# barry-mir/mixing-style-transfer

Hardware: AMD Instinct MI355X
Metric: triplets/sec (10 s @ 44.1 kHz, 4-stem, bs=24) (higher is better)
Workload: dtype f32

## Files before the change

### mixing-style-transfer_amd/csrc/encoder.hip

```cpp
#include "common.h"

#include <cmath>
#include <type_traits>
#include <vector>

namespace {

typedef float f32x4 __attribute__((ext_vector_type(4)));
constexpr int kConvThreads = 512;
constexpr int kConvWaves = 8;

struct FilmParams {
  const float* feats;
  const float *w0t, *b0, *w3t, *b3, *hwt, *hb;
  const float *s1, *t1, *s2, *t2;
  float* film;
  float2* aff1;
  float2* aff2;
  int Fd, H, nsub;
  float* h2;
  int B;
};

constexpr int kFilmCT = 8;
// ... 689 lines not shown
  int nsaddr[4] = {-1, -1, -1, -1};

  auto prefetch_setup = [&](int q, const RTile& t) __attribute__((always_inline)) {
    const int chunk = q % NCH;
    const float* src = p.in + (size_t)t.clip * p.in_clipstride + (size_t)t.band * p.in_bandoff + (size_t)(4 * chunk) * p.in_cstride;
    const float* wsrc = p.wfrag + ((size_t)t.band * NCH + chunk) * WBP;
    nrsrc = __builtin_amdgcn_make_buffer_rsrc(const_cast<float*>(src), 0, (unsigned)(4 * p.in_cstride) * 4u, 0x00020000);
    nwrsrc = __builtin_amdgcn_make_buffer_rsrc(const_cast<float*>(wsrc), 0, (unsigned)WBP * 4u, 0x00020000);
    if (chunk == 0) {
      const bool fold = t.kind == 2;
      const int row0 = (t.kind == 1 ? 4 : 0) - 3, col0 = 16 * t.blk - 3;
      const int rbase = max(row0, 0), cbase = max(col0, 0);
      nsoff = (unsigned)(rbase * p.in_cols + cbase) * 4u;
      int ln = lane;
      asm volatile("" : "+v"(ln));
#pragma unroll
      for (int j = 0; j < 4; ++j) {
        const int e = ln + 64 * j;
        const int r = fold ? e >> 4 : e / PC, c = fold ? e & 15 : e % PC;
        const bool in_patch = fold ? (r < R::FR && c < R::FC) : r < R::PR;
        const int rin = row0 + r, cin = col0 + c;
        const bool ok = t.valid && in_patch && rin >= 0 && rin < p.in_rows && cin >= 0 && cin < p.in_cols;
        nvoff[j] = ok ? (unsigned)((rin - rbase) * p.in_cols + (cin - cbase)) * 4u : 0x80000000u;
        nsaddr[j] = in_patch ? r * PC + c : -1;
      }
    }
  };
  auto prefetch_piece = [&](int i) __attribute__((always_inline)) {
    if (i < NPFK) {
      pf[i] = __builtin_bit_cast(float, __builtin_amdgcn_raw_buffer_load_b32(nrsrc, nvoff[i & 3], nsoff + (unsigned)((i >> 2) * p.in_cstride) * 4u, 0));
    } else if (i < NPIECE) {
      wreg[i - NPFK] = __builtin_bit_cast(f32x4, __builtin_amdgcn_raw_buffer_load_b128(nwrsrc, (unsigned)tid * 16u, (unsigned)(kConvThreads * (i - NPFK)) * 16u, 0));
    }
  };

  f32x4 acc[MT][NT];
  RTile cur{}, nxt{};
  nxt = decode(0);
  if (nq > 0) {
    prefetch_setup(0, nxt);
#pragma unroll
    for (int i = 0; i < NPIECE; ++i) prefetch_piece(i);
  }
#ifdef MST_TRACE
  long long trc[5] = {0, 0, 0, 0, 0};
  const long long trc_start = clock64();
#endif
  for (int q = 0; q < nq; ++q) {
    float* wb = wbuf + (q & 1) * WBP;
#ifdef MST_TRACE
    const long long tq0 = clock64();
#endif
#pragma unroll
    for (int i = 0; i < NWF; ++i) reinterpret_cast<f32x4*>(wb)[tid + kConvThreads * i] = wreg[i];
#pragma unroll
    for (int i = 0; i < NPFK; ++i)
      if (nsaddr[i & 3] >= 0) pbuf[(i >> 2) * CP + nsaddr[i & 3]] = pf[i];
#ifdef MST_TRACE
    asm volatile("s_waitcnt lgkmcnt(0)" ::: "memory");
    const long long tq1 = clock64();
#endif
    __syncthreads();
#ifdef MST_TRACE
    const long long tq2 = clock64();
    trc[0] += tq1 - tq0, trc[1] += tq2 - tq1, trc[4] += 1;
#endif
    cur = nxt;
    if ((q + 1) % NCH == 0) nxt = decode(q + 1);
    prefetch_setup(q + 1, nxt);
    const int chunk = q % NCH;
    if (chunk == 0) {
      ap = cur.kind == 2 ? ap_fold : ap_pair;
#pragma unroll
      for (int t = 0; t < MT; ++t)
#pragma unroll
        for (int n = 0; n < NT; ++n) acc[t][n] = f32x4{0.f, 0.f, 0.f, 0.f};
    }
    {
      float a[2][MT], b[2][NT];
#pragma unroll
      for (int t = 0; t < MT; ++t) a[0][t] = ap[t * PC];
#pragma unroll
      for (int n = 0; n < NT; ++n) b[0][n] = wb[n * 64 + lane];
      auto taps = [&](auto LO_, auto HI_, auto MASK_) __attribute__((always_inline)) {
        constexpr int LO = decltype(LO_)::value, HI = decltype(HI_)::value, MASK = decltype(MASK_)::value;
#pragma unroll
        for (int tap = LO; tap < HI; ++tap) {
          const int cu = tap & 1, nx = cu ^ 1;
          const int off = ((tap + 1) / 7) * PC + ((tap + 1) % 7);
#pragma unroll
          for (int i = 0; i < MT * NT; ++i) {
            const int t = i / NT, n = i % NT;
            if (!((MASK >> t) & 1)) acc[t][n] = __builtin_amdgcn_mfma_f32_16x16x4f32(a[cu][t], b[cu][n], acc[t][n], 0, 0, 0);
            if (tap + 1 < 49) {
              if (i < NT) b[nx][i] = wb[((tap + 1) * NT + i) * 64 + lane];
              else if (i < MT + NT) a[nx][i - NT] = ap[(i - NT) * PC + off];
            }
            if (i >= MT + NT && i - (MT + NT) < PPT) prefetch_piece(tap * PPT + (i - (MT + NT)));
            __builtin_amdgcn_sched_barrier(0);
          }
        }
      };
      using std::integral_constant;
      using I0 = integral_constant<int, 0>;
      using I7 = integral_constant<int, 7>;
      using I14 = integral_constant<int, 14>;
      using I21 = integral_constant<int, 21>;
      using I42 = integral_constant<int, 42>;
      using I49 = integral_constant<int, 49>;
      if (cur.kind == 0) {
        taps(I0{}, I7{}, integral_constant<int, 0b0111>{});
        taps(I7{}, I14{}, integral_constant<int, 0b0011>{});
        taps(I14{}, I21{}, integral_constant<int, 0b0001>{});
      } else {
        taps(I0{}, I21{}, I0{});
      }
      taps(I21{}, I42{}, I0{});
      if (cur.kind == 1) taps(I42{}, I49{}, integral_constant<int, 0b1000>{});
      else taps(I42{}, I49{}, I0{});
    }
#ifdef MST_TRACE
    trc[2] += clock64() - tq2;
#endif
    if (chunk == NCH - 1 && cur.valid) {
      const int j = lane & 15, g = lane >> 4;
      const float2* aff = p.aff + ((size_t)cur.clip * p.nsub + cur.band) * C::COUT;
      const int pr = cur.kind == 2 ? g >> 1 : cur.kind;
      const int pc = 4 * cur.blk + (cur.kind == 2 ? g & 1 : g);
#pragma unroll
      for (int n = 0; n < NT; ++n) {
        const int ch = n * 16 + j;
        const float2 ac = aff[ch];
        float m = 0.f;
#pragma unroll
        for (int t = 0; t < MT; ++t)
#pragma unroll
          for (int r = 0; r < 4; ++r) m = fmaxf(m, fmaf(acc[t][n][r], ac.x, ac.y));
        if (pc < p.out_cols)
          p.out[(((size_t)cur.clip * p.nsub + cur.band) * C::COUT + ch) * p.out_rows * p.out_cols + (size_t)pr * p.out_cols + pc] = m;
      }
    }
  }
#ifdef MST_TRACE
  if (lane == 0 && p.yraw) {
    float* o = p.yraw + (blockIdx.x * kConvWaves + wave) * 8;
    for (int i = 0; i < 5; ++i) o[i] = (float)trc[i];
    o[5] = (float)(clock64() - trc_start);
  }
#endif
}

template <int SUB>
constexpr size_t kConv1ResidentLds = (size_t)(2 * 49 * CC<1, SUB>::NT * 64 + kConvWaves * 8 * CC<1, SUB>::PR * CC<1, SUB>::PC) * sizeof(float);
template <int SUB, int MODE = 0, int LAY = 0>
__global__ __launch_bounds__(kConvThreads) void conv1_resident_kernel(const ConvParams p) {
  using C = CC<1, SUB>;
  constexpr int MT = C::MT, NT = C::NT, PR = C::PR, PC = C::PC;
  static_assert(C::RL == 64, "resident conv1 expects one loader row per instruction");
  static_assert(LAY == 0 || PR == 8, "the channel-minor loader maps lane bits 1..3 to the 8 patch rows");
  constexpr int WCH = 49 * NT * 64;
  constexpr int WBP = ConvGeom<1, SUB>::WBP;
  constexpr int CHS = PR * PC;
  constexpr int PATCH = 8 * CHS;
  constexpr int NPF = LAY == 0 ? 8 * PR : (PC + 3) / 4;
  extern __shared__ __attribute__((aligned(16))) float smem[];
  const int tid = threadIdx.x, lane = tid & 63;
  const int wave = __builtin_amdgcn_readfirstlane(tid >> 6);
  float* wres = smem;
  float* pbuf = smem + 2 * WCH + wave * PATCH;
  constexpr bool DYN = MODE == 0;
  constexpr int kTickets = 16;
  __shared__ unsigned tickets[kTickets];
#ifdef MST_TRACE
  long long trc[5] = {0, 0, 0, 0, 0};
  const long long trc_start = clock64();
#endif

  const int G = gridDim.x;
  const int wg = mst::xcd_remap(blockIdx.x, G);
  const int total_sets = (p.clip_major ? (p.B + p.clip_major - 1) / p.clip_major : 1) * p.nsub * p.sets_per_band;
  const int s_begin = (int)((long long)wg * total_sets / G), s_end = (int)((long long)(wg + 1) * total_sets / G);
  const int tpb = p.tiles_r * p.tiles_c;

  auto decode = [&](int s) __attribute__((always_inline)) {
    Tile t;
    int ti;
    if (p.clip_major) {
      const int ngrp = (p.B + p.clip_major - 1) / p.clip_major;
      const int gb = min(s / p.sets_per_band, ngrp * p.nsub - 1);
      const int idx = (s - gb * p.sets_per_band) * kConvWaves + wave;
      const int grp = gb / p.nsub, c0 = grp * p.clip_major;
      t.band = gb - grp * p.nsub;
      t.valid = (s < s_end) && idx < min(p.clip_major, p.B - c0) * tpb;
      const int cl = t.valid ? idx / tpb : 0;
      t.clip = c0 + cl;
      ti = t.valid ? idx - cl * tpb : 0;
    } else {
      t.band = min(s / p.sets_per_band, p.nsub - 1);
      const int idx = (s - t.band * p.sets_per_band) * kConvWaves + wave;
      t.valid = (s < s_end) && idx < p.B * tpb;
      t.clip = t.valid ? idx / tpb : 0;
      ti = t.valid ? idx - t.clip * tpb : 0;
    }
    t.tc = ti / p.tiles_r;
    t.tr = ti - t.tc * p.tiles_r;
    return t;
  };

  const int kq = lane >> 4, ai = lane & 15, ag = ai >> 2, areg = ai & 3;
  int abase[MT];
#pragma unroll
  for (int t = 0; t < MT; ++t) {
    const int e = 4 * t + areg, wv = e / C::WIN, pos = e % C::WIN;
    abase[t] = kq * CHS + (pos / 5) * PC + 5 * (C::WPG * ag + wv) + pos % 5;
  }

  typename std::conditional<LAY == 0, float, f32x4>::type pf[NPF];
  unsigned long long rowmask = 0;
  bool col_ok = false;
  int coff = 0, nrow0 = 0, nvalid = 0;
  const float* nsrc = p.in;
  bool nfast = false;
  __amdgpu_buffer_rsrc_t nrsrc = __builtin_amdgcn_make_buffer_rsrc(const_cast<float*>(p.in), 0, 0, 0x00020000);
  unsigned nsoff = 0, nvoff = 0;
  static_assert(WBP - WCH >= 4, "the chunk pitch leaves at least 16 zero bytes behind the weights");
  const float* const zero16 = p.wfrag + WCH;
  const int lr = (lane >> 1) & 7, lhalf = lane & 1, lfq = lane >> 4;
  const unsigned frame_bytes = (unsigned)p.cm_mels * 32u;
  auto prefetch_setup = [&](const Tile& t) __attribute__((always_inline)) {
    nrow0 = C::TROWS * t.tr - 3;
    nvalid = t.valid;
    rowmask = 0;
    if constexpr (LAY == 0) {
      const int col0 = C::TCOLS * t.tc - 3, cin = col0 + lane;
      nsrc = p.in + (size_t)t.clip * p.in_clipstride + (size_t)t.band * p.in_bandoff;
      col_ok = lane < PC && cin >= 0 && cin < p.in_cols;
      coff = min(max(cin, 0), p.in_cols - 1);
    } else {
      const int rin = nrow0 + lr, rc = min(max(rin, 0), p.in_rows - 1);
      nsrc = p.in + (size_t)t.clip * p.in_clipstride;
      col_ok = nvalid && rin == rc;
      coff = ((t.band * p.cm_overlap + rc) * 8 + 4 * lhalf) * 4;
      nrow0 = C::TCOLS * t.tc - 3 + lfq;
      if constexpr (DYN) {
        const int f0 = C::TCOLS * t.tc - 3;
        nfast = nvalid && f0 >= 0 && f0 + 4 * NPF + 3 < p.in_cols;
        nrsrc = __builtin_amdgcn_make_buffer_rsrc(const_cast<float*>(nsrc), 0, (unsigned)p.in_cols * frame_bytes, 0x00020000);
        nsoff = (unsigned)max(f0, 0) * frame_bytes;
        nvoff = col_ok ? (unsigned)coff + (unsigned)lfq * frame_bytes : 0x80000000u;
      }
    }
  };
  auto prefetch_piece = [&](int i) __attribute__((always_inline)) {
    if (i < NPF) {
      if constexpr (LAY == 0) {
        const int cc = i / PR, r = i % PR;
        const int rin = nrow0 + r;
        const int rc = min(max(rin, 0), p.in_rows - 1);
        if (nvalid && rin == rc) rowmask |= 1ull << i;
        const float* rowp = nsrc + (size_t)cc * p.in_cstride + (size_t)rc * p.in_cols;
        if constexpr (DYN) pf[i] = (nvalid && rin == rc && col_ok) ? rowp[coff] : *zero16;
        else pf[i] = rowp[coff];
      } else {
        const int fin = nrow0 + 4 * i, fc = min(max(fin, 0), p.in_cols - 1);
        if (col_ok && fin == fc) rowmask |= 1ull << i;
        if (DYN && nfast) {
          pf[i] = __builtin_bit_cast(f32x4, __builtin_amdgcn_raw_buffer_load_b128(nrsrc, nvoff, nsoff + (unsigned)(4 * i) * frame_bytes, 0));
        } else {
          const unsigned boff = (unsigned)fc * frame_bytes + (unsigned)coff;
          const char* src = reinterpret_cast<const char*>(nsrc) + boff;
          if constexpr (DYN) src = (col_ok && fin == fc) ? src : reinterpret_cast<const char*>(zero16);
          pf[i] = *reinterpret_cast<const f32x4*>(src);
        }
      }
    }
  };
  auto prefetch_step = [&](int ks) __attribute__((always_inline)) {
    if constexpr (LAY == 0) prefetch_piece(ks);
    else if (ks % 8 == 0) prefetch_piece(ks / 8);
  };

  f32x4 acc[MT][NT];
  double st[NT][2];
#pragma unroll
  for (int n = 0; n < NT; ++n) st[n][0] = st[n][1] = 0.0;
  int cur_band = -1;
  const int spb = p.sets_per_band;
  const int gb0 = s_begin / spb, nseg = s_end > s_begin ? (s_end - 1) / spb - gb0 + 1 : 0;
  int dseg = 0, dlo = 0, dhi = 0, dgb = 0, nxt_seg = 0;
  auto seg_range = [&](int k) __attribute__((always_inline)) {
    dgb = gb0 + k;
    const int cm = p.clip_major ? p.clip_major : p.B, grp = p.clip_major ? dgb / p.nsub : 0;
    dlo = max(s_begin - dgb * spb, 0) * kConvWaves;
    dhi = min((min(s_end, (dgb + 1) * spb) - dgb * spb) * kConvWaves, min(cm, p.B - grp * cm) * tpb);
  };
  unsigned tkv = 0;
  auto ticket_issue = [&]() __attribute__((always_inline)) {
    tkv = 0;
    if (dseg < nseg && lane == 0)
      tkv = __hip_atomic_fetch_add(&tickets[dseg % kTickets], 1u, __ATOMIC_RELAXED, __HIP_MEMORY_SCOPE_WORKGROUP);
  };
  auto ticket_take = [&]() __attribute__((always_inline)) {
    Tile t{};
    while (dseg < nseg) {
      const int idx = dlo + (int)__builtin_amdgcn_readfirstlane(tkv);
      if (idx < dhi) {
        const int grp = p.clip_major ? dgb / p.nsub : 0;
        const int cl = idx / tpb, ti = idx - cl * tpb;
        t.valid = 1;
        t.band = dgb - grp * p.nsub;
        t.clip = grp * p.clip_major + cl;
        t.tc = ti / p.tiles_r;
        t.tr = ti - t.tc * p.tiles_r;
        return t;
      }
      if (++dseg < nseg) seg_range(dseg);
      ticket_issue();
    }
    return t;
  };
  Tile cur{}, nxt{};
  if constexpr (DYN) {
    if (tid < kTickets) tickets[tid] = 0;
    __syncthreads();
    if (nseg > 0) seg_range(0);
    ticket_issue();
    nxt = ticket_take();
    nxt_seg = dseg;
  } else {
    nxt = decode(s_begin);
  }
  prefetch_setup(nxt);
#pragma unroll
  for (int i = 0; i < NPF; ++i) prefetch_piece(i);

  auto mask_piece = [&](int i) __attribute__((always_inline)) {
    if constexpr (LAY == 0) {
      pf[i] = (((rowmask >> i) & 1ull) && col_ok) ? pf[i] : 0.f;
    } else {
      const bool ok = (rowmask >> i) & 1ull;
#pragma unroll
      for (int k = 0; k < 4; ++k) pf[i][k] = ok ? pf[i][k] : 0.f;
    }
  };
  auto stage_ = [&](auto MASKED_) __attribute__((always_inline)) {
    constexpr bool MASKED = decltype(MASKED_)::value;
    if constexpr (LAY == 0) {
#pragma unroll
      for (int i = 0; i < NPF; ++i) {
        if (!MASKED) mask_piece(i);
        if (lane < PC) pbuf[i * PC + lane] = pf[i];
      }
    } else {
      float* pl = pbuf + (4 * lhalf) * CHS + lr * PC + lfq;
#pragma unroll
      for (int i = 0; i < NPF; ++i) {
        if (4 * i + 3 < PC || 4 * i + lfq < PC) {
          if (!MASKED) mask_piece(i);
#pragma unroll
          for (int k = 0; k < 4; ++k) pl[k * CHS + 4 * i] = pf[i][k];
        }
      }
    }
  };
  auto stage = [&]() __attribute__((always_inline)) { stage_(std::false_type{}); };
  auto tile_body = [&]() __attribute__((always_inline)) {
#ifdef MST_TRACE
    const long long tr0 = clock64();
#endif
#pragma unroll
    for (int t = 0; t < MT; ++t)
#pragma unroll
      for (int n = 0; n < NT; ++n) acc[t][n] = f32x4{0.f, 0.f, 0.f, 0.f};
    {
      float a[2][MT], b[2][NT];
#pragma unroll
      for (int t = 0; t < MT; ++t) a[0][t] = pbuf[abase[t]];
#pragma unroll
      for (int n = 0; n < NT; ++n) b[0][n] = wres[n * 64 + lane];
#pragma unroll
      for (int ks = 0; ks < 98; ++ks) {
        const int cu = ks & 1, nx = cu ^ 1;
        const int tap = (ks + 1) >> 1, ch = (ks + 1) & 1;
        const int off = ch * 4 * CHS + (tap / 7) * PC + (tap % 7);
#pragma unroll
        for (int i = 0; i < MT * NT; ++i) {
          const int t = i / NT, n = i % NT;
          acc[t][n] = __builtin_amdgcn_mfma_f32_16x16x4f32(a[cu][t], b[cu][n], acc[t][n], 0, 0, 0);
          if (ks + 1 < 98) {
            if (i < NT) b[nx][i] = wres[ch * WCH + (tap * NT + i) * 64 + lane];
            else if (i < MT + NT) a[nx][i - NT] = pbuf[abase[i - NT] + off];
          }
          if (i == MT + NT) prefetch_step(ks);
          __builtin_amdgcn_sched_barrier(0);
        }
      }
    }
#ifdef MST_TRACE
    const long long tr1 = clock64();
    trc[0] += tr1 - tr0, trc[4] += 1;
#endif
    if constexpr (MODE == 1) {
      const int j = lane & 15, g = lane >> 4;
      float* yb = p.yraw + ((((size_t)cur.clip * p.nsub + cur.band) * p.acc_tr + cur.tr) * p.acc_tc + cur.tc) *
                               (size_t)(NT * 64 * 4 * MT);
#pragma unroll
      for (int n = 0; n < NT; ++n) {
        const float b = p.bias[cur.band * C::COUT + n * 16 + j];
        f32x4* dst = reinterpret_cast<f32x4*>(yb) + (size_t)n * (64 * MT) + lane;
#pragma unroll
        for (int t = 0; t < MT; ++t) {
          f32x4 v = acc[t][n];
#pragma unroll
          for (int r = 0; r < 4; ++r) {
            v[r] += b;
            const int e = 4 * t + r, wv = e / C::WIN, pos = e % C::WIN;
            const int col = C::TCOLS * cur.tc + 5 * (C::WPG * g + wv) + pos % 5;
            if (col < p.raw_cols) st[n][0] += (double)v[r], st[n][1] += (double)v[r] * (double)v[r];
          }
          dst[64 * t] = v;
        }
      }
    } else
    {
      const int j = lane & 15, g = lane >> 4;
      const float2* aff = p.aff + ((size_t)cur.clip * p.nsub + cur.band) * C::COUT;
      float* orow = p.out + ((size_t)cur.clip * p.nsub + cur.band) * C::COUT * p.out_rows * p.out_cols +
                    (size_t)cur.tr * p.out_cols;
#pragma unroll
      for (int n = 0; n < NT; ++n) {
        const int ch = n * 16 + j;
        const float2 ac = aff[ch];
#pragma unroll
        for (int wv = 0; wv < C::WPG; ++wv) {
          const int pc = 4 * C::WPG * cur.tc + C::WPG * g + wv;
          if (SUB == 2 && p.pool_h == 1) {
#pragma unroll
            for (int hr = 0; hr < 2; ++hr) {
              float m = 0.f;
#pragma unroll
              for (int pos = 0; pos < 5; ++pos) {
                const int e = wv * C::WIN + 5 * hr + pos;
                m = fmaxf(m, fmaf(acc[e >> 2][n][e & 3], ac.x, ac.y));
              }
              if (pc < p.out_cols && 2 * cur.tr + hr < p.out_rows)
                orow[(size_t)ch * p.out_rows * p.out_cols + (size_t)(cur.tr + hr) * p.out_cols + pc] = m;
            }
          } else {
            float m = 0.f;
#pragma unroll
            for (int pos = 0; pos < C::WIN; ++pos) {
              const int e = wv * C::WIN + pos;
              m = fmaxf(m, fmaf(acc[e >> 2][n][e & 3], ac.x, ac.y));
            }
            if (pc < p.out_cols) orow[(size_t)ch * p.out_rows * p.out_cols + pc] = m;
          }
        }
      }
    }
#ifdef MST_TRACE
    trc[1] += clock64() - tr1;
#endif
  };
  f32x4 sav[MT][NT];
  float2 sav_ac[NT];
  Tile prev{};
#pragma unroll
  for (int t = 0; t < MT; ++t)
#pragma unroll
    for (int n = 0; n < NT; ++n) sav[t][n] = f32x4{0.f, 0.f, 0.f, 0.f};
#pragma unroll
  for (int n = 0; n < NT; ++n) sav_ac[n] = float2{0.f, 0.f};
  auto epi_part = [&](auto N_, auto WV_) __attribute__((always_inline)) {
    constexpr int n = decltype(N_)::value, wv = decltype(WV_)::value;
    const int j = lane & 15, g = lane >> 4;
    const int ch = n * 16 + j;
    float* orow = p.out + ((size_t)prev.clip * p.nsub + prev.band) * C::COUT * p.out_rows * p.out_cols + (size_t)prev.tr * p.out_cols;
    const float2 ac = sav_ac[n];
    const int pc = 4 * C::WPG * prev.tc + C::WPG * g + wv;
    if (SUB == 2 && p.pool_h == 1) {
#pragma unroll
      for (int hr = 0; hr < 2; ++hr) {
        float m = 0.f;
#pragma unroll
        for (int pos = 0; pos < 5; ++pos) {
          const int e = wv * C::WIN + 5 * hr + pos;
          m = fmaxf(m, fmaf(sav[e >> 2][n][e & 3], ac.x, ac.y));
        }
        if (prev.valid && pc < p.out_cols && 2 * prev.tr + hr < p.out_rows)
          orow[(size_t)ch * p.out_rows * p.out_cols + (size_t)(prev.tr + hr) * p.out_cols + pc] = m;
      }
    } else {
      float m = 0.f;
#pragma unroll
      for (int pos = 0; pos < C::WIN; ++pos) {
        const int e = wv * C::WIN + pos;
        m = fmaxf(m, fmaf(sav[e >> 2][n][e & 3], ac.x, ac.y));
      }
      if (prev.valid && pc < p.out_cols) orow[(size_t)ch * p.out_rows * p.out_cols + pc] = m;
    }
  };
  auto tile_dyn = [&]() __attribute__((always_inline)) {
#ifdef MST_TRACE
    const long long tr0 = clock64();
#endif
    float2 e_ac[NT];
    {
      const float2* aff = p.aff + ((size_t)cur.clip * p.nsub + cur.band) * C::COUT;
#pragma unroll
      for (int n = 0; n < NT; ++n) e_ac[n] = aff[n * 16 + (lane & 15)];
    }
    {
      constexpr int kEpi0 = 12;
      const bool skip_c = cur.tr == 0, skip_b = 2 * cur.tr + 2 >= p.in_rows;
      const int next_off = skip_b ? 0 : 5 * PC, next_w = skip_b ? 0 : 35 * NT * 64;
      float a[2][MT], b[2][NT];
#pragma unroll
      for (int t = 0; t < MT; ++t) a[0][t] = pbuf[abase[t] + 2 * PC];
#pragma unroll
      for (int n = 0; n < NT; ++n) b[0][n] = wres[(14 * NT + n) * 64 + lane];
      auto kstep = [&](auto S_) __attribute__((always_inline)) {
        constexpr int ks = decltype(S_)::value;
        constexpr int cu = ks & 1, nx = cu ^ 1;
        constexpr bool last = ks == 41 || ks == 69 || ks == 97;
        constexpr int s1 = ks + 1, l1 = s1 < 42 ? s1 : s1 < 70 ? s1 - 42 : s1 - 70;
        constexpr int row1 = (s1 < 42 ? 2 : s1 < 70 ? 5 : 0) + l1 / 14, tap1 = 7 * row1 + (l1 % 14) / 2, ch1 = l1 & 1;
        constexpr int off1 = ch1 * 4 * CHS + row1 * PC + (l1 % 14) / 2;
#pragma unroll
        for (int i = 0; i < MT * NT; ++i) {
          const int t = i / NT, n = i % NT;
          acc[t][n] = __builtin_amdgcn_mfma_f32_16x16x4f32(a[cu][t], b[cu][n], ks == 0 ? f32x4{0.f, 0.f, 0.f, 0.f} : acc[t][n], 0, 0, 0);
          if constexpr (!last) {
            if (i < NT) b[nx][i] = wres[ch1 * WCH + (tap1 * NT + i) * 64 + lane];
            else if (i < MT + NT) a[nx][i - NT] = pbuf[abase[i - NT] + off1];
          } else if constexpr (ks == 41) {
            if (i < NT) b[nx][i] = wres[next_w + i * 64 + lane];
            else if (i < MT + NT) a[nx][i - NT] = pbuf[abase[i - NT] + next_off];
          } else if constexpr (ks == 69) {
            if (i < NT) b[nx][i] = wres[i * 64 + lane];
            else if (i < MT + NT) a[nx][i - NT] = pbuf[abase[i - NT]];
          }
          if (i == MT + NT) {
            if constexpr (LAY == 0) {
              if constexpr (ks >= 8 && ks < 8 + NPF / 2) prefetch_piece(2 * (ks - 8)), prefetch_piece(2 * (ks - 8) + 1);
            } else {
              if constexpr (ks >= 8 && ks % 2 == 0 && ks / 2 - 4 < NPF) prefetch_piece(ks / 2 - 4);
            }
          }
          if (i == MT + NT + 1) {
            if constexpr (ks == 0) ticket_issue();
            if constexpr (ks == 6) {
              nxt = ticket_take();
              nxt_seg = dseg;
              prefetch_setup(nxt);
            }
            if constexpr (ks >= kEpi0 && ks < kEpi0 + 2 * NT * C::WPG && (ks - kEpi0) % 2 == 0)
              epi_part(std::integral_constant<int, (ks - kEpi0) / 2 / C::WPG>{}, std::integral_constant<int, (ks - kEpi0) / 2 % C::WPG>{});
          }
          __builtin_amdgcn_sched_barrier(0);
        }
      };
      static_assert(LAY == 0 ? 8 + NPF / 2 <= 42 : 2 * (NPF + 3) < 42, "the patch fetch must fit block A");
      static_for<42>([&](auto I) __attribute__((always_inline)) { kstep(std::integral_constant<int, decltype(I)::value>{}); });
      if (!skip_b) static_for<28>([&](auto I) __attribute__((always_inline)) { kstep(std::integral_constant<int, 42 + decltype(I)::value>{}); });
      if (!skip_c) static_for<28>([&](auto I) __attribute__((always_inline)) { kstep(std::integral_constant<int, 70 + decltype(I)::value>{}); });
    }
    {
      const float bz = wres[lane];
#pragma unroll
      for (int t = 0; t < MT; ++t)
#pragma unroll
        for (int n = 0; n < NT; ++n) sav[t][n] = __builtin_amdgcn_mfma_f32_16x16x4f32(0.f, bz, acc[t][n], 0, 0, 0);
    }
#pragma unroll
    for (int n = 0; n < NT; ++n) sav_ac[n] = e_ac[n];
    prev = cur;
#ifdef MST_TRACE
    trc[0] += clock64() - tr0, trc[4] += 1;
#endif
  };
  auto load_band = [&](int band) __attribute__((always_inline)) {
    for (int c = 0; c < 2; ++c) {
      const f32x4* src = reinterpret_cast<const f32x4*>(p.wfrag + ((size_t)band * 2 + c) * WBP);
      for (int k = tid; k < WCH / 4; k += kConvThreads) reinterpret_cast<f32x4*>(wres + c * WCH)[k] = src[k];
    }
  };
  if constexpr (DYN) {
    for (int k = 0; k < nseg; ++k) {
#ifdef MST_TRACE
      const long long tb0 = clock64();
#endif
      __syncthreads();
      load_band((gb0 + k) % p.nsub);
      if (tid == 0) tickets[(k + kTickets - 1) % kTickets] = 0;
      __syncthreads();
#ifdef MST_TRACE
      trc[3] += clock64() - tb0;
#endif
      while (nxt.valid && nxt_seg == k) {
#ifdef MST_TRACE
        const long long ts0 = clock64();
#endif
        cur = nxt;
#ifdef MST_TRACE
        asm volatile("s_waitcnt vmcnt(0)" ::: "memory");
        const long long ts1 = clock64();
        trc[1] += ts1 - ts0;
#endif
        stage_(std::true_type{});
#ifdef MST_TRACE
        asm volatile("s_waitcnt lgkmcnt(0)" ::: "memory");
        trc[2] += clock64() - ts1;
#endif
        tile_dyn();
      }
    }
    {
      static_for<NT * C::WPG>([&](auto I) __attribute__((always_inline)) {
        constexpr int q = decltype(I)::value;
        epi_part(std::integral_constant<int, q / C::WPG>{}, std::integral_constant<int, q % C::WPG>{});
      });
    }
#ifdef MST_TRACE
    if (lane == 0 && p.yraw) {
      float* o = p.yraw + (blockIdx.x * kConvWaves + wave) * 8;
      for (int i = 0; i < 5; ++i) o[i] = (float)trc[i];
      o[5] = (float)(clock64() - trc_start);
    }
#endif
  } else {
  for (int s = s_begin; s < s_end; ++s) {
    cur = nxt;
    if (cur.band != cur_band) {
      if (MODE == 1 && cur_band >= 0) flush_stats<NT, C::COUT>(st, p.stats, cur_band, lane);
      __syncthreads();
      load_band(cur.band);
      __syncthreads();
      cur_band = cur.band;
    }
    stage();
    nxt = decode(s + 1);
    prefetch_setup(nxt);
    if (!cur.valid) {
#pragma unroll
      for (int i = 0; i < NPF; ++i) prefetch_piece(i);
      continue;
    }
    tile_body();
  }
  }
  if (MODE == 1 && cur_band >= 0) flush_stats<NT, C::COUT>(st, p.stats, cur_band, lane);
}

__global__ __launch_bounds__(256) void absmax_kernel(const float* __restrict__ x, long long n_per_clip, unsigned* out) {
  const float* base = x + (size_t)blockIdx.y * n_per_clip;
  float m = 0.f;
  const long long n4 = n_per_clip >> 2;
  const float4* b4 = reinterpret_cast<const float4*>(base);
  const bool al = (reinterpret_cast<uintptr_t>(base) & 15) == 0;
  if (al) {
    for (long long i = (long long)blockIdx.x * 256 + threadIdx.x; i < n4; i += (long long)gridDim.x * 256) {
      const float4 v = b4[i];
      m = fmaxf(fmaxf(m, fmaxf(fabsf(v.x), fabsf(v.y))), fmaxf(fabsf(v.z), fabsf(v.w)));
    }
    for (long long i = (n4 << 2) + (long long)blockIdx.x * 256 + threadIdx.x; i < n_per_clip; i += (long long)gridDim.x * 256)
      m = fmaxf(m, fabsf(base[i]));
  } else {
    for (long long i = (long long)blockIdx.x * 256 + threadIdx.x; i < n_per_clip; i += (long long)gridDim.x * 256)
      m = fmaxf(m, fabsf(base[i]));
  }
  m = mst::wave_max(m);
  if ((threadIdx.x & 63) == 0) atomicMax(out + blockIdx.y, __float_as_uint(m));
}

__global__ __launch_bounds__(64) void f16_scale_kernel(const float2* __restrict__ aff1, const float* __restrict__ w1norm,
                                                        const unsigned* __restrict__ xmax_bits, float* scale, int nsub,
                                                        const float* __restrict__ bias = nullptr, float gain = 1.0f) {
  const int clip = blockIdx.x / nsub, band = blockIdx.x % nsub, c = threadIdx.x & 31;
  const float xmax = __uint_as_float(xmax_bits[clip]);
  const float2 a = aff1[((size_t)clip * nsub + band) * 32 + c];
  float bound = fmaf(fabsf(a.x), fmaf(w1norm[band * 32 + c], xmax, bias ? fabsf(bias[band * 32 + c]) : 0.f), fabsf(a.y)) * gain;
  bound = mst::wave_max(bound);
  if (threadIdx.x == 0) {
    int k = 0;
    if (bound > 0.f && bound < INFINITY) {
      int ex;
      (void)frexpf(bound, &ex);
      k = max(-60, min(60, 14 - ex));
    } else if (!(bound < INFINITY)) {
      k = -60;
    }
    scale[(size_t)blockIdx.x * 2] = ldexpf(1.0f, k);
    scale[(size_t)blockIdx.x * 2 + 1] = ldexpf(1.0f, -k);
  }
}

typedef _Float16 h16x8 __attribute__((ext_vector_type(8)));
__device__ __forceinline__ _Float16 to_f16_sat(float v) {
  return (_Float16)(__builtin_isfinite(v) ? fminf(fmaxf(v, -65504.f), 65504.f) : v);
}
constexpr int kF16Steps = 13;

template <int SUB>
constexpr size_t kConv1F16Lds = (size_t)(kF16Steps * CC<1, SUB>::NT * 2 * 64 + kConvWaves * 2 * CC<1, SUB>::PR * CC<1, SUB>::PC) * 16;
template <int SUB, int TERMS, int MODE = 0, int LAY = 0>
__global__ __launch_bounds__(kConvThreads) void conv1_f16x3_kernel(const ConvParams p, const h16x8* __restrict__ wfrag16,
                                                                  _Float16* __restrict__ out_hi, _Float16* __restrict__ out_lo) {
  using C = CC<1, SUB>;
  constexpr int MT = C::MT, NT = C::NT, PR = C::PR, PC = C::PC;
  static_assert(C::RL == 64, "one loader row per instruction");
  static_assert(LAY == 0 || (LAY == 2 && PR == 8), "the channel-minor loader maps lane bits 0..2 to the 8 patch rows");
  constexpr int WVEC = kF16Steps * NT * 2 * 64;
  constexpr int PVEC = PR * PC;
  constexpr int NPF = LAY == 0 ? 8 * PR : (PC + 7) / 8;
  extern __shared__ __attribute__((aligned(16))) float smem[];
  const int tid = threadIdx.x, lane = tid & 63;
  const int wave = __builtin_amdgcn_readfirstlane(tid >> 6);
  h16x8* wres = reinterpret_cast<h16x8*>(smem);
// ... 2177 lines not shown
  if (rc) {
    mst_encoder_destroy(e);
    return rc;
  }
  *out = e;
  return MST_OK;
}

void mst_encoder_destroy(mst_encoder* e) {
  if (!e) return;
  for (void* q : e->owned) (void)hipFree(q);
  delete e;
}

int mst_encoder_set_precision(mst_encoder* e, int conv1_f16x3) {
  MST_REQUIRE(e, "mst_encoder_set_precision: NULL encoder");
  MST_REQUIRE(conv1_f16x3 == 0 || (conv1_f16x3 >= 1 && conv1_f16x3 <= 3 && (e->sub == 2 || (e->sub == 1 && e->cfg.split_size % 2 == 0))),
              "mst_encoder_set_precision: the f16 modes (1, 2, 3) need 2-row conv1 tiles (20-mel sub-bands, or an even split_size below 20)");
  e->conv1_f16x3 = conv1_f16x3;
  return MST_OK;
}

int mst_encoder_set_train_precision(mst_encoder* e, int f16_operands) {
  MST_REQUIRE(e, "mst_encoder_set_train_precision: NULL encoder");
  MST_REQUIRE(f16_operands == 0 || ((f16_operands == 1 || f16_operands == 2) && (e->sub == 2 || e->cfg.split_size % 2 == 0)),
              "mst_encoder_set_train_precision: modes 1 (f16 operands) and 2 (split precision) need 2-row conv1 tiles (20-mel sub-bands, or an even split_size below 20)");
  if (f16_operands && !e->w2dfrag16) {
    const size_t ns = e->cfg.n_subbands;
    int rc = enc_alloc(e, &e->f16_wsc2d, ns * 32);
    if (!rc) rc = enc_alloc(e, &e->f16_winv2d, ns * 32);
    if (!rc) rc = enc_alloc(e, &e->w2dfrag16, ns * 8 * kF16Steps * 2 * 2 * 64 * 8);
    if (rc) return rc;
  }
  e->train_f16 = f16_operands;
  return MST_OK;
}

size_t mst_encoder_workspace_bytes(const mst_encoder* e, int B, int frames) {
  if (!e || B <= 0 || frames < 20) return 0;
  return ws_layout(e, B, frames).total;
}

static bool conv1_resident_geometry(const mst_encoder* e) {
  return (e->sub == 2 || (e->sub == 1 && e->cfg.split_size % 2 == 0)) && !getenv("MST_CONV1_CHUNKED");
}

int mst_encoder_layout_supported(const mst_encoder* e, int layout) {
  if (!e) return 0;
  if (layout == MST_LOGMEL_REF) return 1;
  if (e->sub > 2) return 0;
  if (layout == MST_LOGMEL_CM32) return e->conv1_f16x3 == 0 && conv1_resident_geometry(e);
  if (layout == MST_LOGMEL_CM16) return e->conv1_f16x3 != 0;
  return 0;
}

int mst_encoder_forward(const mst_encoder* e, const float* logmel, int frames, const float* feats, int B, float* emb,
                        const mst_encoder_taps* taps, void* workspace, size_t workspace_bytes, void* stream) {
  mst_logmel_in in{};
  in.layout = MST_LOGMEL_REF, in.data = logmel;
  return mst_encoder_forward_in(e, &in, frames, feats, B, emb, taps, workspace, workspace_bytes, stream);
}

int mst_encoder_forward_in(const mst_encoder* e, const mst_logmel_in* lin, int frames, const float* feats, int B, float* emb,
                           const mst_encoder_taps* taps, void* workspace, size_t workspace_bytes, void* stream) {
  MST_REQUIRE(e && lin && lin->data && feats && emb, "mst_encoder_forward: NULL argument");
  const int lay = lin->layout;
  if (const int rc = check_logmel_in("mst_encoder_forward", lin, mst_encoder_layout_supported(e, lay), e->conv1_f16x3,
                                     e->conv1_f16x3 != 3, e->conv1_f16x3 >= 2))
    return rc;
  const float* logmel = static_cast<const float*>(lin->data);
  MST_REQUIRE(B > 0 && frames >= 20, "mst_encoder_forward: need B>0 and frames>=20 (B=%d frames=%d)", B, frames);
  const WsLayout L = ws_layout(e, B, frames);
  MST_REQUIRE(L.W2 >= 1, "mst_encoder_forward: clip too short for two pooling stages (frames=%d)", frames);
  if (!workspace || workspace_bytes < L.total)
    return mst::fail(MST_ENOMEM, "mst_encoder_forward: workspace %zu B < required %zu B", workspace_bytes, L.total);
  hipStream_t st = reinterpret_cast<hipStream_t>(stream);
  char* ws = reinterpret_cast<char*>(workspace);
  const int ns = e->cfg.n_subbands;
  float* film = (taps && taps->film) ? taps->film : reinterpret_cast<float*>(ws + L.film);
  float* pool1 = (taps && taps->pool1) ? taps->pool1 : reinterpret_cast<float*>(ws + L.pool1);
  float* pool_in = (taps && taps->pool_in) ? taps->pool_in : reinterpret_cast<float*>(ws + L.pool_in);
  float2* aff1 = reinterpret_cast<float2*>(ws + L.aff1);
  float2* aff2 = reinterpret_cast<float2*>(ws + L.aff2);
  auto mark = [&](int i) {
    if (taps && taps->events[i]) (void)hipEventRecord(reinterpret_cast<hipEvent_t>(taps->events[i]), st);
  };
  mark(0);
  MST_HIP_CHECK(launch_film(film_params(e, feats, film, aff1, aff2, reinterpret_cast<float*>(ws + L.film_h2), B), st));
  mark(1);
  const int grid = e->num_cus;
  const dim3 blk(kConvThreads);
  {
    ConvParams cp{};
    cp.in = logmel, cp.wfrag = e->w1frag, cp.aff = aff1, cp.out = pool1, cp.B = B, cp.nsub = ns;
    conv1_input_geometry(cp, e, frames);
    cp.in_lo = lin->lo, cp.cm_mels = e->cfg.n_mels, cp.cm_overlap = e->cfg.overlap;
    cp.out_rows = e->H1, cp.out_cols = L.W1;
    cp.tiles_r = e->H1;
    cp.tiles_c = e->sub == 2 ? (L.W1 + 7) / 8 : (L.W1 + 15) / 16;
    const bool resident = e->sub <= 2 && !e->conv1_f16x3 && conv1_resident_geometry(e);
    if (e->sub == 1 && (e->conv1_f16x3 || resident)) {
      cp.pool_h = 1;
      cp.tiles_r = e->cfg.split_size / 2;
      cp.tiles_c = (L.W1 + 7) / 8;
    }
    cp.sets_per_band = sets_per_band(B, cp.tiles_r, cp.tiles_c);
    const int g = std::min(grid, ns * cp.sets_per_band);
    hipError_t err;
    if (e->sub > 2) {
      MST_REQUIRE(lay == MST_LOGMEL_REF && e->conv1_f16x3 == 0, "mst_encoder_forward: split_size=%d runs in the reference layout, fp32 only", e->cfg.split_size);
      err = mst::launch_lds<conv1_generic_kernel>(dim3((L.W1 + kGenCols - 1) / kGenCols, B * ns), dim3(256),
                                                  conv1_generic_lds(e->cfg.split_size), st, cp, e->sub);
    } else if (e->conv1_f16x3) {
      const bool both = e->conv1_f16x3 >= 2;
      cp.f16_winv = e->f16_winv1;
      if (both && !(taps && taps->pool1)) cp.out = nullptr;
      if (both) {
        const unsigned* xmax = lin->absmax;
        float* fsc = reinterpret_cast<float*>(ws + L.f16scale);
        if (!xmax) {
          unsigned* xm = reinterpret_cast<unsigned*>(ws + L.xmax);
          MST_HIP_CHECK(hipMemsetAsync(xm, 0, (size_t)B * sizeof(unsigned), st));
          const long long npc = (long long)8 * e->cfg.n_mels * frames;
          hipLaunchKernelGGL(absmax_kernel, dim3(64, B), dim3(256), 0, st, logmel, npc, xm);
          xmax = xm;
        }
        hipLaunchKernelGGL(f16_scale_kernel, dim3(B * ns), dim3(64), 0, st, aff1, e->w1norm, xmax, fsc, ns);
        cp.f16_scale = fsc;
      }
      const h16x8* wf = reinterpret_cast<const h16x8*>(e->w1frag16);
      _Float16* oh = both ? reinterpret_cast<_Float16*>(ws + L.pool1_h16) : nullptr;
      _Float16* ol = e->conv1_f16x3 == 2 ? reinterpret_cast<_Float16*>(ws + L.pool1_l16) : nullptr;
      if (lay == MST_LOGMEL_CM16) {
        const h16x8* wfe = reinterpret_cast<const h16x8*>(e->w1frag16e);
        if (e->conv1_f16x3 == 3) {
          cp.sets_per_band = sets_per_band(B, cp.tiles_r, cp.tiles_c, kF16eWaves<1>);
          const int g1 = std::min(grid, ns * cp.sets_per_band);
          err = mst::launch_lds<conv1_f16e_kernel<1>>(dim3(g1), dim3(kF16eWaves<1> * 64), kConv1F16eLds<1>, st, cp, wfe, oh, ol);
        }
        else err = mst::launch_lds<conv1_f16e_kernel<3>>(dim3(g), blk, kConv1F16eLds<3>, st, cp, wfe, oh, ol);
      } else if (e->conv1_f16x3 == 3) err = mst::launch_lds<conv1_f16x3_kernel<2, 1>>(dim3(g), blk, kConv1F16Lds<2>, st, cp, wf, oh, ol);
      else err = mst::launch_lds<conv1_f16x3_kernel<2, 3>>(dim3(g), blk, kConv1F16Lds<2>, st, cp, wf, oh, ol);
    } else if (resident) {
      if (!getenv("MST_CONV1_BAND_MAJOR")) {
        const char* env = getenv("MST_CONV1_CLIP_GROUP");
        cp.clip_major = std::max(1, std::min(B, env ? atoi(env) : 1));
        cp.sets_per_band = sets_per_band(cp.clip_major, cp.tiles_r, cp.tiles_c);
      }
      const int g = std::min(grid, (cp.clip_major ? (B + cp.clip_major - 1) / cp.clip_major : 1) * ns * cp.sets_per_band);
#ifdef MST_TRACE
      static ConvTrace trace;
      trace_attach(trace, cp);
#endif
      if (lay == MST_LOGMEL_CM32) err = mst::launch_lds<conv1_resident_kernel<2, 0, 1>>(dim3(g), blk, kConv1ResidentLds<2>, st, cp);
      else err = mst::launch_lds<conv1_resident_kernel<2>>(dim3(g), blk, kConv1ResidentLds<2>, st, cp);
#ifdef MST_TRACE
      trace_dump(trace, g, false);
#endif
    } else {
      err = e->sub == 2 ? launch_conv<1, 2>(cp, g, st) : launch_conv<1, 1>(cp, g, st);
    }
    if (err != hipSuccess) return mst::fail(MST_EHIP, "conv1 launch failed: %s", hipGetErrorString(err));
  }
  mark(2);
  {
    ConvParams cp{};
    cp.in = pool1, cp.wfrag = e->w2frag, cp.aff = aff2, cp.out = pool_in, cp.B = B, cp.nsub = ns;
    conv2_input_geometry(cp, e, L.W1);
    cp.out_rows = e->FD, cp.out_cols = L.W2;
    cp.tiles_r = (e->FD + 1) / 2;
    cp.tiles_c = (L.W2 + 1) / 2;
    cp.sets_per_band = sets_per_band(B, cp.tiles_r, cp.tiles_c);
    const int g = std::min(grid, ns * cp.sets_per_band);
    hipError_t err;
    if (e->conv1_f16x3 >= 2) {
      cp.f16_scale = reinterpret_cast<const float*>(ws + L.f16scale);
      cp.f16_winv = e->f16_winv2;
      const h16x8* ih = reinterpret_cast<const h16x8*>(ws + L.pool1_h16);
      const h16x8* il = reinterpret_cast<const h16x8*>(ws + L.pool1_l16);
      const h16x8* wf = reinterpret_cast<const h16x8*>(e->w2frag16);
      if (e->conv1_f16x3 == 3) err = mst::launch_lds<conv2_f16x3_kernel<1>>(dim3(g), blk, kConv2F16Lds, st, cp, ih, il, wf);
      else err = mst::launch_lds<conv2_f16x3_kernel<3>>(dim3(g), blk, kConv2F16Lds, st, cp, ih, il, wf);
    } else {
#ifdef MST_TRACE
      static ConvTrace trace;
      trace_attach(trace, cp);
#endif
      const char* tiles_env = getenv("MST_CONV2_TILES");
      if (e->FD == 2 && e->H1 == 10 && !(tiles_env && !strcmp(tiles_env, "8x8"))) {
        const int rem = L.W2 % 4;
        cp.rt_blocks = L.W2 / 4 + (rem == 3);
        cp.rt_fold = rem == 1 || rem == 2;
        cp.rt_pair_sets = (B * cp.rt_blocks + 3) / 4;
        cp.sets_per_band = cp.rt_pair_sets + (B * cp.rt_fold + kConvWaves - 1) / kConvWaves;
        err = mst::launch_lds<conv2_rows_kernel>(dim3(std::min(grid, ns * cp.sets_per_band)), blk, RowTiles::kLds, st, cp);
      } else {
        err = launch_conv<2, 2>(cp, g, st);
      }
#ifdef MST_TRACE
      trace_dump(trace, g, true);
#endif
    }
    if (err != hipSuccess) return mst::fail(MST_EHIP, "conv2 launch failed: %s", hipGetErrorString(err));
  }
  mark(3);
  if (const int rc = launch_head(e, L, ws, pool_in, emb, B, st, taps ? taps->events[4] : nullptr)) return rc;
  mark(5);
  return MST_OK;
}

namespace {
struct TrainLayout {
  WsLayout base;
  size_t y1, y2, stats1, stats2, bn1, bn2, dfilm_acc, dw_acc, total;
  size_t t_pool1_h16, t_pool1_l16, t_f16scale, t_xmax, t_bscale, t_dyg1, t_dyg2, t_ys1, t_ys2;
  int tr1, tc1, tr2, tc2;
};
TrainLayout train_layout(const mst_encoder* e, int B, int frames) {
  TrainLayout T{};
  T.base = ws_layout(e, B, frames);
  const int ns = e->cfg.n_subbands;
  const bool two_row = e->sub == 2 || train_fwd16(e);
  const int tcols1 = two_row ? 40 : 80;
  T.tr1 = two_row ? e->cfg.split_size / 2 : e->H1, T.tc1 = (frames + tcols1 - 1) / tcols1;
  T.tr2 = (e->H1 + 7) / 8, T.tc2 = (T.base.W1 + 7) / 8;
  size_t o = T.base.total;
  auto take = [&](size_t bytes) {
    const size_t at = o;
    o += mst::align_up(bytes, 256);
    return at;
  };
  const size_t ybytes = e->train_f16 == 1 ? 2 : 4;
  T.y1 = take((size_t)B * ns * T.tr1 * T.tc1 * 2 * 64 * 20 * ybytes);
  T.y2 = take((size_t)B * ns * T.tr2 * T.tc2 * 4 * 64 * 16 * ybytes);
  T.stats1 = take((size_t)(ns * 32 * 2 + 1) * sizeof(mst::DetAcc));
  T.stats2 = take((size_t)(ns * 64 * 2 + 1) * sizeof(mst::DetAcc));
  T.bn1 = take((size_t)ns * 32 * 8);
  T.bn2 = take((size_t)ns * 64 * 8);
  T.dfilm_acc = take((size_t)B * ns * 192 * sizeof(mst::DetAcc));
  T.dw_acc = take((size_t)ns * 64 * 1568 * sizeof(mst::DetAcc));
  const size_t f = train_fwd16(e) ? 1 : 0, fb = train_bwd16(e) ? 1 : 0;
  T.t_pool1_h16 = take(f * (size_t)B * ns * 32 * e->H1 * T.base.W1 * 2);
  T.t_pool1_l16 = take((e->train_f16 == 2 ? 1 : 0) * (size_t)B * ns * 32 * e->H1 * T.base.W1 * 2);
  T.t_f16scale = take(f * (size_t)B * ns * 2 * 4);
  T.t_xmax = take(f * (size_t)B * 4);
  T.t_ys1 = take((e->train_f16 == 1 ? 1 : 0) * (size_t)ns * 2 * 4);
  T.t_ys2 = take((e->train_f16 == 1 ? 1 : 0) * (size_t)ns * 2 * 4);
  T.t_bscale = take(fb * 16);
  const size_t cgs = (size_t)((B + 7) / 8);
  const size_t hl = e->train_f16 == 2 ? 2 : 1;
  T.t_dyg1 = take(fb * hl * (size_t)ns * cgs * T.tr1 * T.tc1 * 2 * 20 * 64 * 16);
  T.t_dyg2 = take(fb * hl * (size_t)ns * cgs * T.tr2 * T.tc2 * 4 * 16 * 64 * 16);
  T.total = o;
  return T;
}
}

size_t mst_encoder_train_workspace_bytes(const mst_encoder* e, int B, int frames) {
  if (!e || B <= 0 || frames < 20 || e->sub > 2) return 0;
  return train_layout(e, B, frames).total;
}

int mst_encoder_train_stats_buffer(const mst_encoder* e, int layer, int B, int frames, size_t* offset_bytes, size_t* n_int64) {
  MST_REQUIRE(e && offset_bytes && n_int64 && (layer == 1 || layer == 2) && B > 0 && frames >= 20,
              "mst_encoder_train_stats_buffer: bad arguments");
  const TrainLayout T = train_layout(e, B, frames);
  *offset_bytes = layer == 1 ? T.stats1 : T.stats2;
  *n_int64 = ((size_t)e->cfg.n_subbands * (layer == 1 ? 32 : 64) * 2 + 1) * (sizeof(mst::DetAcc) / 8);
  return MST_OK;
}

int mst_encoder_train_scale_buffer(const mst_encoder* e, int B, int frames, size_t* offset_bytes) {
  MST_REQUIRE(e && offset_bytes && B > 0 && frames >= 20, "mst_encoder_train_scale_buffer: bad arguments");
  MST_REQUIRE(train_bwd16(e), "mst_encoder_train_scale_buffer: the fp32 training mode has no internal loss scale");
  *offset_bytes = train_layout(e, B, frames).t_bscale + 2 * sizeof(float);
  return MST_OK;
}

int mst_encoder_train_layout_supported(const mst_encoder* e, int layout) {
  if (!e) return 0;
  if (layout == MST_LOGMEL_REF) return 1;
  if (layout == MST_LOGMEL_CM16) return train_fwd16(e) ? 1 : 0;
  return 0;
}

int mst_encoder_forward_train(const mst_encoder* e, const float* logmel, int frames, const float* feats, int B, float* emb,
                              const mst_encoder_train_taps* taps, void* workspace, size_t workspace_bytes, void* stream) {
  mst_logmel_in in{};
  in.layout = MST_LOGMEL_REF, in.data = logmel;
  return mst_encoder_forward_train_in(e, &in, frames, feats, B, emb, taps, workspace, workspace_bytes, stream);
}

int mst_encoder_forward_train_in(const mst_encoder* e, const mst_logmel_in* lin, int frames, const float* feats, int B, float* emb,
                                 const mst_encoder_train_taps* taps, void* workspace, size_t workspace_bytes, void* stream) {
  MST_REQUIRE(e && e->sub <= 2, "mst_encoder_forward_train: the training kernels cover first-pool heights 1 and 2 (split_size < 30)");
  MST_REQUIRE(e && lin && lin->data && (feats || (taps && taps->film_in)), "mst_encoder_forward_train: NULL argument");
  const int lay = lin->layout;
  if (const int rc = check_logmel_in("mst_encoder_forward_train", lin, mst_encoder_train_layout_supported(e, lay), e->train_f16,
                                     e->train_f16 != 1, false))
    return rc;
  const float* logmel = static_cast<const float*>(lin->data);
  MST_REQUIRE(B > 0 && frames >= 20, "mst_encoder_forward_train: need B>0 and frames>=20 (B=%d frames=%d)", B, frames);
  const TrainLayout T = train_layout(e, B, frames);
  const WsLayout& L = T.base;
  MST_REQUIRE(L.W2 >= 1, "mst_encoder_forward_train: clip too short for two pooling stages (frames=%d)", frames);
  if (!workspace || workspace_bytes < T.total)
    return mst::fail(MST_ENOMEM, "mst_encoder_forward_train: workspace %zu B < required %zu B", workspace_bytes, T.total);
  hipStream_t st = reinterpret_cast<hipStream_t>(stream);
// ... 768 lines not shown
```

Before: 2835.

## Reorder conv1 M-tiles row-pure and skip MFMAs on padded boundary rows

Adds a row-pure element ordering for the resident conv1 kernel so that each 4-element M-tile covers a single input row. At the top and bottom image edges, tiles that read only zero-padded rows can then skip their MFMAs and patch loads through compile-time masks. It also changes the buffer-load offset to an incrementing scalar register, kept opaque to the compiler with an empty asm. The row-pure variant becomes the default, with an env var to restore the old mixed order. This adds more template instantiations and code size, and the epilogue index remap has to stay consistent with the new order.

```diff
diff --git a/mixing-style-transfer_amd/csrc/encoder.hip b/mixing-style-transfer_amd/csrc/encoder.hip
--- a/mixing-style-transfer_amd/csrc/encoder.hip
+++ b/mixing-style-transfer_amd/csrc/encoder.hip
@@ -865,9 +865,10 @@
 
 template <int SUB>
 constexpr size_t kConv1ResidentLds = (size_t)(2 * 49 * CC<1, SUB>::NT * 64 + kConvWaves * 8 * CC<1, SUB>::PR * CC<1, SUB>::PC) * sizeof(float);
-template <int SUB, int MODE = 0, int LAY = 0>
+template <int SUB, int MODE = 0, int LAY = 0, int RP = 0>
 __global__ __launch_bounds__(kConvThreads) void conv1_resident_kernel(const ConvParams p) {
   using C = CC<1, SUB>;
+  static_assert(RP == 0 || (MODE == 0 && SUB == 2), "the row-pure order belongs to the eval forward on 2 x 40 tiles");
   constexpr int MT = C::MT, NT = C::NT, PR = C::PR, PC = C::PC;
   static_assert(C::RL == 64, "resident conv1 expects one loader row per instruction");
   static_assert(LAY == 0 || PR == 8, "the channel-minor loader maps lane bits 1..3 to the 8 patch rows");
@@ -924,9 +925,11 @@
   int abase[MT];
 #pragma unroll
   for (int t = 0; t < MT; ++t) {
-    const int e = 4 * t + areg, wv = e / C::WIN, pos = e % C::WIN;
+    const int e = 4 * t + areg;
+    const int wv = RP ? (e / 5) % C::WPG : e / C::WIN, pos = RP ? 5 * (e / (5 * C::WPG)) + e % 5 : e % C::WIN;
     abase[t] = kq * CHS + (pos / 5) * PC + 5 * (C::WPG * ag + wv) + pos % 5;
   }
+  auto elem = [](int wv, int pos) __attribute__((always_inline)) { return RP ? 5 * (C::WPG * (pos / 5) + wv) + pos % 5 : wv * C::WIN + pos; };
 
   typename std::conditional<LAY == 0, float, f32x4>::type pf[NPF];
   unsigned long long rowmask = 0;
@@ -978,12 +981,16 @@
         const int fin = nrow0 + 4 * i, fc = min(max(fin, 0), p.in_cols - 1);
         if (col_ok && fin == fc) rowmask |= 1ull << i;
         if (DYN && nfast) {
-          pf[i] = __builtin_bit_cast(f32x4, __builtin_amdgcn_raw_buffer_load_b128(nrsrc, nvoff, nsoff + (unsigned)(4 * i) * frame_bytes, 0));
+          pf[i] = __builtin_bit_cast(f32x4, __builtin_amdgcn_raw_buffer_load_b128(nrsrc, nvoff, nsoff, 0));
         } else {
           const unsigned boff = (unsigned)fc * frame_bytes + (unsigned)coff;
           const char* src = reinterpret_cast<const char*>(nsrc) + boff;
           if constexpr (DYN) src = (col_ok && fin == fc) ? src : reinterpret_cast<const char*>(zero16);
           pf[i] = *reinterpret_cast<const f32x4*>(src);
+        }
+        if constexpr (DYN) {
+          nsoff += 4u * frame_bytes;
+          asm volatile("" : "+s"(nsoff));
         }
       }
     }
@@ -1197,7 +1204,7 @@
         float m = 0.f;
 #pragma unroll
         for (int pos = 0; pos < 5; ++pos) {
-          const int e = wv * C::WIN + 5 * hr + pos;
+          const int e = elem(wv, 5 * hr + pos);
           m = fmaxf(m, fmaf(sav[e >> 2][n][e & 3], ac.x, ac.y));
         }
         if (prev.valid && pc < p.out_cols && 2 * prev.tr + hr < p.out_rows)
@@ -1207,7 +1214,7 @@
       float m = 0.f;
 #pragma unroll
       for (int pos = 0; pos < C::WIN; ++pos) {
-        const int e = wv * C::WIN + pos;
+        const int e = elem(wv, pos);
         m = fmaxf(m, fmaf(sav[e >> 2][n][e & 3], ac.x, ac.y));
       }
       if (prev.valid && pc < p.out_cols) orow[(size_t)ch * p.out_rows * p.out_cols + pc] = m;
@@ -1232,8 +1239,10 @@
       for (int t = 0; t < MT; ++t) a[0][t] = pbuf[abase[t] + 2 * PC];
 #pragma unroll
       for (int n = 0; n < NT; ++n) b[0][n] = wres[(14 * NT + n) * 64 + lane];
-      auto kstep = [&](auto S_) __attribute__((always_inline)) {
+      auto kstep = [&](auto S_, auto MASK_, auto ZERO_) __attribute__((always_inline)) {
         constexpr int ks = decltype(S_)::value;
+        constexpr int MASK = decltype(MASK_)::value, ZERO = ks == 0 ? (1 << MT) - 1 : decltype(ZERO_)::value;
+        constexpr bool row_end = (ks < 42 ? ks : ks < 70 ? ks - 42 : ks - 70) % 14 == 13;
         constexpr int cu = ks & 1, nx = cu ^ 1;
         constexpr bool last = ks == 41 || ks == 69 || ks == 97;
         constexpr int s1 = ks + 1, l1 = s1 < 42 ? s1 : s1 < 70 ? s1 - 42 : s1 - 70;
@@ -1242,10 +1251,11 @@
 #pragma unroll
         for (int i = 0; i < MT * NT; ++i) {
           const int t = i / NT, n = i % NT;
-          acc[t][n] = __builtin_amdgcn_mfma_f32_16x16x4f32(a[cu][t], b[cu][n], ks == 0 ? f32x4{0.f, 0.f, 0.f, 0.f} : acc[t][n], 0, 0, 0);
+          if (!((MASK >> t) & 1))
+            acc[t][n] = __builtin_amdgcn_mfma_f32_16x16x4f32(a[cu][t], b[cu][n], (ZERO >> t) & 1 ? f32x4{0.f, 0.f, 0.f, 0.f} : acc[t][n], 0, 0, 0);
           if constexpr (!last) {
             if (i < NT) b[nx][i] = wres[ch1 * WCH + (tap1 * NT + i) * 64 + lane];
-            else if (i < MT + NT) a[nx][i - NT] = pbuf[abase[i - NT] + off1];
+            else if (i < MT + NT && (row_end || !((MASK >> (i - NT)) & 1))) a[nx][i - NT] = pbuf[abase[i - NT] + off1];
           } else if constexpr (ks == 41) {
             if (i < NT) b[nx][i] = wres[next_w + i * 64 + lane];
             else if (i < MT + NT) a[nx][i - NT] = pbuf[abase[i - NT] + next_off];
@@ -1274,9 +1284,52 @@
         }
       };
       static_assert(LAY == 0 ? 8 + NPF / 2 <= 42 : 2 * (NPF + 3) < 42, "the patch fetch must fit block A");
-      static_for<42>([&](auto I) __attribute__((always_inline)) { kstep(std::integral_constant<int, decltype(I)::value>{}); });
-      if (!skip_b) static_for<28>([&](auto I) __attribute__((always_inline)) { kstep(std::integral_constant<int, 42 + decltype(I)::value>{}); });
-      if (!skip_c) static_for<28>([&](auto I) __attribute__((always_inline)) { kstep(std::integral_constant<int, 70 + decltype(I)::value>{}); });
+      using std::integral_constant;
+      using NONE = integral_constant<int, 0>;
+      auto steps = [&](auto LO_, auto HI_, auto MASK_) __attribute__((always_inline)) {
+        static_for<decltype(HI_)::value - decltype(LO_)::value>([&](auto I) __attribute__((always_inline)) {
+          kstep(integral_constant<int, decltype(LO_)::value + decltype(I)::value>{}, MASK_, NONE{});
+        });
+      };
+      if constexpr (RP) {
+        using M01 = integral_constant<int, 0b00011>;
+        using M34 = integral_constant<int, 0b11000>;
+        using I0 = integral_constant<int, 0>;
+        using I14 = integral_constant<int, 14>;
+        using I15 = integral_constant<int, 15>;
+        using I28 = integral_constant<int, 28>;
+        using I42 = integral_constant<int, 42>;
+        using I56 = integral_constant<int, 56>;
+        using I70 = integral_constant<int, 70>;
+        using I84 = integral_constant<int, 84>;
+        using I98 = integral_constant<int, 98>;
+        if (cur.tr == 0) {
+          steps(I0{}, I14{}, M01{});
+          kstep(I14{}, NONE{}, M01{});
+        } else {
+          steps(I0{}, I15{}, NONE{});
+        }
+        steps(I15{}, I28{}, NONE{});
+        if (skip_b) steps(I28{}, I42{}, M34{});
+        else steps(I28{}, I42{}, NONE{});
+        if (!skip_b) {
+          steps(I42{}, I56{}, NONE{});
+          if (2 * cur.tr + 4 >= p.in_rows) steps(I56{}, I70{}, M34{});
+          else steps(I56{}, I70{}, NONE{});
+        }
+        if (!skip_c) {
+          if (cur.tr == 1) {
+            steps(I70{}, I84{}, M01{});
+            steps(I84{}, I98{}, NONE{});
+          } else {
+            steps(I70{}, I98{}, NONE{});
+          }
+        }
+      } else {
+        steps(integral_constant<int, 0>{}, integral_constant<int, 42>{}, NONE{});
+        if (!skip_b) steps(integral_constant<int, 42>{}, integral_constant<int, 70>{}, NONE{});
+        if (!skip_c) steps(integral_constant<int, 70>{}, integral_constant<int, 98>{}, NONE{});
+      }
     }
     {
       const float bz = wres[lane];
@@ -3760,8 +3813,15 @@
       static ConvTrace trace;
       trace_attach(trace, cp);
 #endif
-      if (lay == MST_LOGMEL_CM32) err = mst::launch_lds<conv1_resident_kernel<2, 0, 1>>(dim3(g), blk, kConv1ResidentLds<2>, st, cp);
-      else err = mst::launch_lds<conv1_resident_kernel<2>>(dim3(g), blk, kConv1ResidentLds<2>, st, cp);
+      const char* mt = getenv("MST_CONV1_MTILES");
+      const bool mixed = mt && !strcmp(mt, "mixed");
+      if (lay == MST_LOGMEL_CM32) {
+        err = mixed ? mst::launch_lds<conv1_resident_kernel<2, 0, 1, 0>>(dim3(g), blk, kConv1ResidentLds<2>, st, cp)
+                    : mst::launch_lds<conv1_resident_kernel<2, 0, 1, 1>>(dim3(g), blk, kConv1ResidentLds<2>, st, cp);
+      } else {
+        err = mixed ? mst::launch_lds<conv1_resident_kernel<2, 0, 0, 0>>(dim3(g), blk, kConv1ResidentLds<2>, st, cp)
+                    : mst::launch_lds<conv1_resident_kernel<2, 0, 0, 1>>(dim3(g), blk, kConv1ResidentLds<2>, st, cp);
+      }
 #ifdef MST_TRACE
       trace_dump(trace, g, false);
 #endif
```

After: 2854, median of 6. No clear change (+0.7%).
